# yuw444/fastF

Hardware: AMD Instinct MI355X
Metric: BAM records/sec -> deduped UMI matrix; achieved HBM GB/s vs roofline (higher is better)
Workload: dtype u64

## Files before the change

### fastf_amd/csrc/umi_engine.hip

```cpp
#include "umi_kernels.hpp"
#include "sweep_kernels.hpp"
#include "cap_kernels.hpp"

#include <algorithm>
#include <cstdarg>
#include <cstdio>
#include <cstdlib>
#include <cstring>
#include <mutex>
#include <new>
#include <stdexcept>
#include <chrono>
#include <string>
#include <thread>
#include <vector>

extern "C" {
#include "fastf_amd.h"
#include "host_io.h"
#include "mt_jump.h"
}

using namespace fastf;

// ... 173 lines not shown
    u64 batch_cap = 0;
    struct Slot {
        void* h_stage = nullptr;
        void* h_draws = nullptr;
        DevBuf d_stage;
        hipEvent_t ev_copy = nullptr, ev_done = nullptr;
        u64* h_small = nullptr;
        bool busy = false; u64 n = 0; bool external = false;
    } slot[2];
    int cur = 0;
    const u32* cur_umi_ext = nullptr;
    u64 inflight_records = 0;
    u64 key_cap = 0;
    DevBuf d_keys, d_tmp;
    DevBuf d_small;
    u64* h_small = nullptr;
    DevBuf d_feature, d_cell, d_count, d_ukeys, d_ncopy;
    u32* h_coo = nullptr; u64 h_coo_cap = 0, h_nnz = 0;
    bool h_coo_pinned = false; u32 h_coo_uses = 0;
    u32* lent_rows = nullptr; u64 lent_cap = 0;
    u32* rows_at = nullptr; u64 rows_stride = 0;
    std::vector<u32> h_ufeature, h_ucell, h_uumi, h_ncopy;
    std::vector<uint8_t> h_unonnull;
    u64 total_records = 0, hits_so_far = 0, keys_so_far = 0;
    u64 c_sampled = 0, c_valid = 0;
    bool finished = false; int sorted_in_tmp = 0; u64 n_sorted = 0;
    u32 skip_bits = 0;
    bool fully_sorted = false;
    DevBuf d_cellidx, d_tilecnt, d_tilebase, d_binbase, d_cnt;
    DevBuf d_halfhits;
    DevBuf d_segkeys;
    DevBuf d_segcount, d_segprefix, d_tileseg;
    u32 giant_parity = 0;
    u32 seg_n = 0; u64 seg_stride = 0;
    DevBuf d_rgn_phys, d_rgn_hist, d_rgn_blk;
    u32 rgn_hist_n = 0, rgn_hist_shift = 0;
    bool stream_mode = false, store_regions = false;
    bool narrow = false, genes_one_family = false;
    u64 slots_used = 0, slot_cap = 0; u32 rgn_n = 0, rgn_cap = 0;
    DevBuf d_scanblk;
    DevBuf d_rg_feature, d_rg_cell, d_rg_count, d_rg_ukeys, d_spanrows, d_spanbase, d_giant;
    u32 rg_n = 0; bool rg_umi = false;
    bool wide = false, long_umi = false; u32 group_bits = 0;
    u32 sub_bits = 0, row_split = 0;
    bool finish_queued = false;
    DevBuf d_vals, d_vtmp;
    bool timing = false;
    hipEvent_t t_ev[2] = {nullptr, nullptr};
    double t_scatter_ms = 0; u64 t_scatter_n = 0;
    double t_k1_ms = 0; u64 t_k1_n = 0;
    double t_k1b_ms = 0; u64 t_k1b_n = 0;
    double t_k3_ms = 0; u64 t_k3_n = 0;
    double t_count_ms = 0; u64 t_count_n = 0;
    double t_gather_ms = 0; u64 t_gather_n = 0;
};

enum { SM_KEYCOUNT = 0, SM_COUNTERS = 32, SM_NNZ = 64, SM_NROWS_U = 65, SM_N = 66, SM_RUNNING = 96, SM_DRAWBASE = 128, SM_WORDS = 160 };

static int set_scatter_lds_limit();
static u32 g_cu_count = 256;
static int multi_create(const fastf_engine_config_t* cfg, fastf_engine* e);
static void multi_destroy(fastf_engine* e);
static int multi_push(fastf_engine* e, const fastf_batch_t* b, bool pinned);
static int multi_finish(fastf_engine* e, fastf_coo_t* coo, uint64_t counters[3]);
static int multi_umi_rows(fastf_engine* e, fastf_umi_rows_t* rows);
static int multi_reset(fastf_engine* e, bool reseed, u32 seed, u64 skip);
static int multi_device_records(const fastf_engine* e, uint64_t* records, u32 n);
static size_t scatter_smem_bytes(u32 ipt = SORT_IPT) {
    return (size_t)ipt * SORT_THREADS * 8 + (size_t)SORT_WAVES * RADIX * 4 + RADIX * 4 * 2 + 64;
}

static u32 h_slot_hash(u64 key) {
    const u32 h = (u32)key * 0x9E3779B1u + (u32)(key >> 32) * 0x85EBCA77u;
    return h ^ (h >> 15);
}

static int build_table(const u64* keys, u32 n, DevBuf& buf, Table& t, const char* what) {
    u32 cap = 64;
    while (cap < 2ull * n) cap <<= 1;
    std::vector<uint4> slots(cap, make_uint4(0, 0, 0, 0));
    for (u32 i = 0; i < n; ++i) {
        const u64 k = keys[i];
        if (k == 0) return set_err("%s key %u is 0 (unpackable string?)", what, i);
        u32 h = h_slot_hash(k) & (cap - 1);
        for (;;) {
            uint4& s = slots[h];
            const u64 sk = ((u64)s.y << 32) | s.x;
            if (sk == 0) { s.x = (u32)k; s.y = (u32)(k >> 32); s.z = i + 1; break; }
            if (sk == k) return set_err("duplicate %s key at index %u (first occurrence wins in the reference; dedup before create)", what, i);
// ... 248 lines not shown
        int prio_lo = 0, prio_hi = 0;
        const char* sp = getenv("FASTF_STREAM_PRIORITY");
        const bool high = sp && sp[0] == '1' && hipDeviceGetStreamPriorityRange(&prio_lo, &prio_hi) == hipSuccess && prio_hi != prio_lo;
        auto mk = [&](hipStream_t* s) { return high ? hipStreamCreateWithPriority(s, hipStreamNonBlocking, prio_hi) : hipStreamCreateWithFlags(s, hipStreamNonBlocking); };
        if (mk(&e->s_compute) != hipSuccess ||
            mk(&e->s_copy) != hipSuccess ||
            mk(&e->s_mt) != hipSuccess ||
            hipEventCreateWithFlags(&e->ev_mt, hipEventDisableTiming) != hipSuccess ||
            hipEventCreateWithFlags(&e->slot[0].ev_copy, hipEventDisableTiming) != hipSuccess ||
            hipEventCreateWithFlags(&e->slot[1].ev_copy, hipEventDisableTiming) != hipSuccess ||
            hipEventCreateWithFlags(&e->slot[0].ev_done, hipEventDisableTiming) != hipSuccess ||
            hipEventCreateWithFlags(&e->slot[1].ev_done, hipEventDisableTiming) != hipSuccess ||
            hipEventCreate(&e->t_ev[0]) != hipSuccess || hipEventCreate(&e->t_ev[1]) != hipSuccess) {
            rc = set_err("stream/event creation failed"); break;
        }
        lap("streams and events");
        if ((rc = build_table((const u64*)cfg->cell_keys, cfg->n_cells, e->tab_cells, e->cells, "cell"))) break;
        if ((rc = build_table((const u64*)cfg->feature_keys, cfg->n_features, e->tab_feats, e->feats, "feature"))) break;
        {
            const char* lt = getenv("FASTF_LDS_TABLES");
            if (!(lt && lt[0] == '0')) {
                const char* lc = getenv("FASTF_LDS_CELLS");
                if (!(lc && lc[0] == '0') && (rc = build_cell_lds(e, (const u64*)cfg->cell_keys, cfg->n_cells))) break;
                if (!e->use_lds_cells && (rc = build_cell_filter(e, (const u64*)cfg->cell_keys, cfg->n_cells))) break;
                if ((rc = build_gene_lds(e, (const u64*)cfg->feature_keys, cfg->n_features))) break;
            }
        }
        lap("tables built and uploaded");
        if ((rc = e->d_small.ensure(SM_WORDS * sizeof(u64)))) break;
        if (hipHostMalloc((void**)&e->h_small, SM_WORDS * sizeof(u64), hipHostMallocDefault) != hipSuccess) {
            rc = set_err("hipHostMalloc failed"); break;
        }
        if (hipMemset(e->d_small.p, 0, SM_WORDS * sizeof(u64)) != hipSuccess) { rc = set_err("memset failed"); break; }
        lap("counters allocated and cleared");
        if (set_scatter_lds_limit()) {
            rc = set_err("cannot raise dynamic LDS limit to %zu bytes", scatter_smem_bytes()); break;
        }
        lap("kernel attributes (code object loaded)");
        e->batch_cap = cfg->batch_records ? cfg->batch_records : (4ull << 20);
        e->key_cap = cfg->key_capacity;
        e->stream_mode = e->use_lds_genes && !e->wide && e->n_shards == 1 && !getenv("FASTF_NO_STREAM_K1B") && !getenv("FASTF_PUSH_TILE_FORM");
        {
            const char* bw = getenv("FASTF_BLOCK_WIDE");
            e->narrow = e->stream_mode && e->genes_one_family && e->lds_genes.vmin + e->lds_genes.range <= 0xFFFFFFFFull &&
                        e->L.umi_bits <= 24 && !(bw && bw[0] == '1');
        }
    } while (0);
    if (rc) { fastf_engine_destroy(e); return 1; }
    *out = e;
    return 0;
} FASTF_CATCH_INT

extern "C" void fastf_engine_destroy(fastf_engine_t* e) FASTF_TRY {
    if (!e) return;
    if (e->multi) { multi_destroy(e); delete e; return; }
    (void)hipSetDevice(e->device);
    (void)hipDeviceSynchronize();
    for (int i = 0; i < 2; ++i) {
        fastf_engine::Slot& sl = e->slot[i];
        if (sl.h_stage) (void)hipHostFree(sl.h_stage);
        if (sl.h_draws) (void)hipHostFree(sl.h_draws);
        if (sl.h_small) (void)hipHostFree(sl.h_small);
        sl.d_stage.release();
        if (sl.ev_copy) (void)hipEventDestroy(sl.ev_copy);
        if (sl.ev_done) (void)hipEventDestroy(sl.ev_done);
        if (e->t_ev[i]) (void)hipEventDestroy(e->t_ev[i]);
    }
    if (e->h_small) (void)hipHostFree(e->h_small);
    if (e->h_coo) { if (e->h_coo_pinned) pin_unreg(e->h_coo); fastf_big_free(e->h_coo, (size_t)e->h_coo_cap * 12); }
    e->d_ring.release(); e->d_mt.release(); e->d_dbits.release(); e->d_mtwords.release(); e->d_mtsub.release(); e->d_mtpoly.release(); e->d_mtseat.release(); e->d_mtseq.release();
    DevBuf* all[] = {&e->tab_cells, &e->tab_feats, &e->img_cells, &e->img_genes, &e->d_cell_filter, &e->d_keys, &e->d_tmp, &e->d_small, &e->d_feature, &e->d_cell,
                     &e->d_count, &e->d_ukeys, &e->d_ncopy, &e->d_cellidx, &e->d_tilecnt, &e->d_tilebase, &e->d_binbase, &e->d_cnt, &e->d_rg_feature, &e->d_rg_cell, &e->d_rg_count, &e->d_rg_ukeys, &e->d_spanrows, &e->d_spanbase, &e->d_giant, &e->d_scanblk,
                     &e->d_halfhits, &e->d_segcount, &e->d_segprefix, &e->d_tileseg, &e->d_segkeys, &e->d_vals, &e->d_vtmp,
                     &e->d_rgn_phys, &e->d_rgn_hist, &e->d_rgn_blk};
    for (DevBuf* b : all) b->release();
    if (e->s_compute) (void)hipStreamDestroy(e->s_compute);
    if (e->s_copy) (void)hipStreamDestroy(e->s_copy);
    if (e->s_mt) (void)hipStreamDestroy(e->s_mt);
    if (e->ev_mt) (void)hipEventDestroy(e->ev_mt);
    delete e;
} FASTF_CATCH_VOID

extern "C" int fastf_engine_table_modes(const fastf_engine_t* e, int* cells_in_lds, int* genes_in_lds) FASTF_TRY {
    if (!e) return set_err("null engine");
    if (cells_in_lds) *cells_in_lds = e->use_lds_cells;
    if (genes_in_lds) *genes_in_lds = e->use_lds_genes ? (e->lds_genes.direct ? 2 : 1) : 0;
    return 0;
} FASTF_CATCH_INT

extern "C" int fastf_engine_cell_scratch_bytes(const fastf_engine_t* e, uint32_t* bytes) FASTF_TRY {
    if (!e || !bytes) return set_err("null argument");
    *bytes = (e->multi ? e->n_cells <= 65535u : e->cell16) ? 2u : 4u;
    return 0;
} FASTF_CATCH_INT

extern "C" int fastf_engine_sort_passes(const fastf_engine_t* e, uint32_t flags, uint32_t* passes) FASTF_TRY {
    if (!e || !passes) return set_err("null argument");
    *passes = sort_passes(e->L.total_bits, (flags & FASTF_SORT_SKIP_LOW) ? e->skip_bits : 0);
    return 0;
} FASTF_CATCH_INT

extern "C" int fastf_engine_skip_bits(const fastf_engine_t* e, uint32_t* bits) FASTF_TRY {
    if (!e || !bits) return set_err("null argument");
    *bits = e->skip_bits;
    return 0;
} FASTF_CATCH_INT

// ... 455 lines not shown
    p.keys = keys; p.shard_stride = stride; p.key_counts = key_counts; p.counters = counters;
    p.stamps = g_k1_stamps;
    p.n_tiles = tiles;
    p.genes = e->lds_genes;
    p.blk = (const unsigned char*)blk;
    if (e->wide) {
        if (segmented || blk) return set_err("internal error: wide keys take the tile form");
        if (!wide_vals && (e->n_shards != 1 || keys != (u64*)e->d_keys.p)) return set_err("internal error: wide keys go through the engine's own key store");
        p.vals = wide_vals ? wide_vals : (u64*)e->d_vals.p; p.wide_feat_bits = e->feat_bits; p.wide_sub_bits = e->sub_bits;
        p.umi_ext = wide_vals ? wide_ext : e->cur_umi_ext;
    }
    const bool no_stream = getenv("FASTF_NO_STREAM_K1B") != nullptr;
    const bool stream_shards = !segmented && !e->wide && e->n_shards > 1 && e->n_shards <= (u32)MAX_SHARDS && e->use_lds_genes && !no_stream;
    if (blk && !(segmented || stream_shards)) return set_err("FASTF_PROBE_BLOCKED needs the streaming K1b (fastf_dev_block_bytes returns 0 otherwise)");
    t_begin(e, s);
    if (segmented || stream_shards) {
        u32 grid; u64 region;
        stream_geometry(e, tiles, &grid, &region);
        const u32 n_rgn = grid * (u32)K1S_SUB, rgn0 = app ? app->rgn0 : 0u;
        if (stream_shards) {
            if (e->d_segkeys.ensure((size_t)n_rgn * region * sizeof(u64))) return 1;
            p.keys = (u64*)e->d_segkeys.p;
        } else if ((u64)n_rgn * region > stride) return set_err("segmented key output needs %llu slots, the buffer has %llu (fastf_dev_probe_capacity)",
                                                                (unsigned long long)((u64)n_rgn * region), (unsigned long long)stride);
        if (app) {
            if (e->rgn_cap < rgn0 + n_rgn) return set_err("internal error: region tables too small");
        } else {
            if (e->rgn_n) return set_err("device-level K1 on an engine that holds pushed chunks: fastf_engine_reset first");
            if (grow_regions(e, n_rgn)) return 1;
        }
        if (e->d_segprefix.ensure(((size_t)n_rgn + 1) * sizeof(u64))) return 1;
        StreamParams sp{(const u32*)e->d_halfhits.p, region, (u64*)e->d_segcount.p + rgn0,
                        stream_shards ? nullptr : (u32*)e->d_rgn_hist.p + (size_t)rgn0 * RADIX, (u64*)e->d_rgn_phys.p + rgn0,
                        app ? app->slot0 : 0ull, e->skip_bits};
        const int variant = (e->genes_blocks_per_cu >= 2 ? 0 : 4) | (e->cell16 ? 2 : 0) | (e->lds_genes.direct ? 1 : 0);
#define FPS(R, C, D) do { if (blk && e->narrow) hipLaunchKernelGGL((filter_pack_stream_kernel<R, C, D, true, true>), dim3(grid), dim3(R ? K1S_THREADS_ROOMY : K1S_THREADS), e->lds_genes.bytes, s, p, sp); \
                          else if (blk) hipLaunchKernelGGL((filter_pack_stream_kernel<R, C, D, true>), dim3(grid), dim3(R ? K1S_THREADS_ROOMY : K1S_THREADS), e->lds_genes.bytes, s, p, sp); \
                          else hipLaunchKernelGGL((filter_pack_stream_kernel<R, C, D, false>), dim3(grid), dim3(R ? K1S_THREADS_ROOMY : K1S_THREADS), e->lds_genes.bytes, s, p, sp); } while (0)
        switch (variant) {
        case 0: FPS(false, false, false); break; case 1: FPS(false, false, true); break;
        case 2: FPS(false, true, false); break;  case 3: FPS(false, true, true); break;
        case 4: FPS(true, false, false); break;  case 5: FPS(true, false, true); break;
        case 6: FPS(true, true, false); break;   default: FPS(true, true, true); break;
        }
#undef FPS
        if (stream_shards) {
            hipLaunchKernelGGL(shard_partition_kernel, dim3(n_rgn), dim3(SP_THREADS), 0, s, (const u64*)e->d_segkeys.p, (const u64*)e->d_segcount.p,
                               region, e->L.cell_shift, e->n_shards, keys, stride, key_counts, counters + 3);
        } else if (app) {
            hipLaunchKernelGGL(seg_scan_kernel, dim3(1), dim3(1024), 0, s, (const u64*)e->d_segcount.p + rgn0, n_rgn, (u64*)e->d_segprefix.p, key_counts, true);
        } else {
            hipLaunchKernelGGL(seg_scan_kernel, dim3(1), dim3(1024), 0, s, (const u64*)e->d_segcount.p, n_rgn, (u64*)e->d_segprefix.p, key_counts, false);
            e->seg_n = n_rgn; e->seg_stride = region;
            e->rgn_hist_n = n_rgn; e->rgn_hist_shift = e->skip_bits;
        }
    } else if (e->use_lds_genes) {
        const u32 grid = std::min<u32>(tiles, e->genes_blocks_per_cu * g_cu_count);
        if (e->genes_blocks_per_cu >= 2) hipLaunchKernelGGL((filter_pack_kernel<true, false>), dim3(grid), dim3(K1B_THREADS), e->lds_genes.bytes, s, p);
        else hipLaunchKernelGGL((filter_pack_kernel<true, true>), dim3(grid), dim3(K1B_THREADS), e->lds_genes.bytes, s, p);
    } else {
        hipLaunchKernelGGL(filter_pack_kernel<false>, dim3(tiles), dim3(K1B_THREADS), 0, s, p);
    }
    HIP_OK(hipGetLastError());
    t_end(e, s, &e->t_k1b_ms, &e->t_k1b_n);
    dbg_sync(s, blk ? "K1b filter_pack (blocked)" : "K1b filter_pack");
    return 0;
}

extern "C" int fastf_dev_probe_pack(fastf_engine_t* e, const uint64_t* d_cb_key, const uint64_t* d_gx_key,
                                    const uint32_t* d_umi, const uint32_t* d_meta, uint64_t n,
                                    const uint32_t* d_draws, uint64_t n_draws, const uint64_t* d_draw_base,
                                    uint64_t* d_keys_out, uint64_t shard_stride, uint64_t* d_key_counts,
                                    uint64_t* d_counters, uint32_t flags, void* stream) FASTF_TRY {
    if (!e) return set_err("null engine");
    if (e->multi) return set_err("fastf_dev_probe_pack: device-level calls take a single-device engine");
    HIP_OK(hipSetDevice(e->device));
    NO_WIDE(e, "fastf_dev_probe_pack");
    const bool seg = (flags & FASTF_PROBE_SEGMENTED) != 0, blocked = (flags & FASTF_PROBE_BLOCKED) != 0;
    if (seg && !(e->n_shards == 1 && e->use_lds_genes))
        return set_err("FASTF_PROBE_SEGMENTED needs a single shard and the gene table in LDS (fastf_dev_probe_capacity returns 0 otherwise)");
    if (blocked && !d_gx_key) return set_err("FASTF_PROBE_BLOCKED: d_gx_key must point at the blocked buffer");
    if (n && n_draws && !d_draws) return set_err("null d_draws");
    if (!(flags & FASTF_PROBE_DRAW_BITS) && n && n_draws) {
        if (e->d_dbits.ensure(((n_draws + 63) / 64) * 8)) return 1;
        if (launch_draw_bits(e->threshold, d_draws, n_draws, (u32*)e->d_dbits.p, (hipStream_t)stream)) return 1;
        d_draws = (const uint32_t*)e->d_dbits.p;
// ... 73 lines not shown

static int set_scatter_lds_limit() {
    const void* fns[10] = {(const void*)scatter_kernel<0>, (const void*)scatter_kernel<8>, (const void*)scatter_kernel<16>,
                           (const void*)scatter_kernel<24>, (const void*)scatter_kernel<32>, (const void*)scatter_kernel<40>,
                           (const void*)scatter_kernel<48>, (const void*)scatter_kernel<56>, (const void*)scatter_kernel<-1>,
                           (const void*)scatter_kernel<-1, true>};
    for (const void* f : fns)
        if (hipFuncSetAttribute(f, hipFuncAttributeMaxDynamicSharedMemorySize, (int)scatter_smem_bytes()) != hipSuccess) return 1;
    if (hipFuncSetAttribute((const void*)scatter_kernel<-1, false, true>, hipFuncAttributeMaxDynamicSharedMemorySize, (int)scatter_smem_bytes_vals(SORT_IPT)) != hipSuccess) return 1;
    if (hipFuncSetAttribute((const void*)scatter_regions_kernel, hipFuncAttributeMaxDynamicSharedMemorySize, (int)scatter_smem_bytes()) != hipSuccess) return 1;
    return 0;
}

static int launch_sort(fastf_engine* e, u64* keys, u64* tmp, const u64* d_n, u64 max_n, u32 key_bits, u32 low_bit,
                       int* sorted_in_tmp, hipStream_t s, bool segmented_input = false, u64* vals = nullptr, u64* vtmp = nullptr) {
    if (key_bits > 64) return set_err("key_bits %u > 64", key_bits);
    const u32 passes = sort_passes(key_bits, low_bit);
    *sorted_in_tmp = (int)(passes & 1);
    if (max_n == 0) return 0;
    if (max_n >= (1ull << 32)) return set_err("sort of %llu keys: limit is 2^32-1 per shard", (unsigned long long)max_n);
    if (reserve_workspace(e, 0, max_n)) return 1;
    const u32 ipt = choose_sort_ipt(max_n);
    const u32 T = (u32)((max_n + (u64)ipt * SORT_THREADS - 1) / ((u64)ipt * SORT_THREADS));
    u32* bintot = (u32*)e->d_binbase.p; u32* cnt = (u32*)e->d_cnt.p;
    SegMap seg{nullptr, nullptr, 0, 0};
    bool walk = false;
    if (segmented_input) {
        if (!e->seg_n) return set_err("FASTF_SORT_SEGMENTED without a preceding FASTF_PROBE_SEGMENTED probe_pack");
        if (passes == 0) return set_err("segmented keys need at least one sort pass");
        static const bool no_walk = getenv("FASTF_NO_REGION_WALK") != nullptr;
        walk = e->rgn_hist_n == e->seg_n && e->rgn_hist_shift == low_bit && !no_walk && !vals;
        if (!walk) {
            if (!e->seg_stride) return set_err("internal error: regions without a common stride need their histograms");
            seg = SegMap{(const u64*)e->d_segprefix.p, (const TileSeg*)e->d_tileseg.p, e->seg_n, e->seg_stride};
            hipLaunchKernelGGL(seg_tiles_kernel, dim3(std::min<u32>((T + 255) / 256, 1024)), dim3(256), 0, s, seg.prefix, seg.n_seg,
                               seg.stride, ipt * SORT_THREADS, (TileSeg*)e->d_tileseg.p);
        }
    }
    const SegMap none{nullptr, nullptr, 0, 0};
    for (u32 q = 0; q < passes; ++q) {
        const u64* src = (q & 1) ? tmp : keys;
        u64* dst = (q & 1) ? keys : tmp;
        const u32 shift = low_bit + 8 * q;
        if (q == 0 && walk) {
            const u32 R = e->seg_n, n_blk = (R + RGN_BLK - 1) / RGN_BLK;
            if (e->d_rgn_blk.ensure((size_t)n_blk * RADIX * sizeof(u32))) return 1;
            hipLaunchKernelGGL(rgn_scan_blocks_kernel, dim3(n_blk), dim3(RADIX), 0, s, (u32*)e->d_rgn_hist.p, R, (u32*)e->d_rgn_blk.p);
            hipLaunchKernelGGL(rgn_scan_fix_kernel, dim3(n_blk), dim3(RADIX), 0, s, (u32*)e->d_rgn_hist.p, R, (const u32*)e->d_rgn_blk.p, n_blk, bintot);
            t_begin(e, s);
            hipLaunchKernelGGL(scatter_regions_kernel, dim3(tile_grid(R)), dim3(SORT_THREADS), scatter_smem_bytes(ipt), s, src, dst,
                               (const u64*)e->d_rgn_phys.p, (const u64*)e->d_segcount.p, (const u32*)e->d_rgn_hist.p, (const u32*)bintot, R, ipt, shift,
                               max_n >= (24ull << 20));
            t_end(e, s, &e->t_scatter_ms, &e->t_scatter_n);
            e->rgn_hist_n = 0;
            dbg_sync(s, "K2 sort pass (region walk)");
            continue;
        }
        t_begin(e, s);
        if (q == 0 && seg.prefix) hipLaunchKernelGGL(tile_count_kernel<true>, dim3(tile_grid(T)), dim3(SORT_THREADS), 0, s, src, d_n, shift, cnt, ipt, seg);
        else hipLaunchKernelGGL(tile_count_kernel<false>, dim3(tile_grid(T)), dim3(SORT_THREADS), 0, s, src, d_n, shift, cnt, ipt, none);
        t_end(e, s, &e->t_count_ms, &e->t_count_n);
        hipLaunchKernelGGL(row_scan_kernel, dim3(RADIX), dim3(1024), 0, s, cnt, d_n, bintot, ipt);
        t_begin(e, s);
        if (vals) launch_scatter(shift, T, s, src, dst, d_n, (const u32*)cnt, (const u32*)bintot, ipt, none, (q & 1) ? vtmp : vals, (q & 1) ? vals : vtmp);
        else launch_scatter(shift, T, s, src, dst, d_n, (const u32*)cnt, (const u32*)bintot, ipt, q == 0 ? seg : none);
        t_end(e, s, &e->t_scatter_ms, &e->t_scatter_n);
        dbg_sync(s, "K2 sort pass");
    }
    HIP_OK(hipGetLastError());
    return 0;
}

extern "C" int fastf_dev_set_regions(fastf_engine_t* e, const uint64_t* d_counts, uint32_t n_regions, uint64_t stride,
                                     uint64_t* d_n_out, void* stream) FASTF_TRY {
    if (!e || !d_counts || !d_n_out) return set_err("null argument");
    if (e->multi) return set_err("fastf_dev_set_regions: device-level calls take a single-device engine");
    if (n_regions == 0 || stride == 0) return set_err("fastf_dev_set_regions: no regions");
    HIP_OK(hipSetDevice(e->device));
    if (e->d_segprefix.ensure(((size_t)n_regions + 1) * sizeof(u64))) return 1;
    hipLaunchKernelGGL(seg_scan_kernel, dim3(1), dim3(1024), 0, (hipStream_t)stream, (const u64*)d_counts, (u32)n_regions, (u64*)e->d_segprefix.p, (u64*)d_n_out);
    HIP_OK(hipGetLastError());
    e->seg_n = n_regions; e->seg_stride = stride; e->rgn_hist_n = 0;
    return 0;
} FASTF_CATCH_INT

extern "C" int fastf_dev_sort(fastf_engine_t* e, uint64_t* d_keys, uint64_t* d_tmp, const uint64_t* d_n,
                              uint64_t max_n, uint32_t key_bits, uint32_t flags, int* sorted_in_tmp, void* stream) FASTF_TRY {
    if (!e) return set_err("null engine");
    if (e->multi) return set_err("fastf_dev_sort: device-level calls take a single-device engine");
    NO_WIDE(e, "fastf_dev_sort");
    HIP_OK(hipSetDevice(e->device));
    int dummy = 0;
    return launch_sort(e, (u64*)d_keys, (u64*)d_tmp, (const u64*)d_n, max_n, key_bits,
                       (flags & FASTF_SORT_SKIP_LOW) ? e->skip_bits : 0,
                       sorted_in_tmp ? sorted_in_tmp : &dummy, (hipStream_t)stream, (flags & FASTF_SORT_SEGMENTED) != 0);
} FASTF_CATCH_INT

static u32 k3_grid(u64 max_n, int dedup) {
    static int per_cu[3] = {-1, -1, -1};
    if (per_cu[dedup] < 0) {
        const char* c = getenv("FASTF_K3_PER_CU");
        per_cu[dedup] = c ? atoi(c) : 4;
        if (per_cu[dedup] < 1) per_cu[dedup] = 1;
    }
    const u64 tiles = (max_n + K3_TILE - 1) / K3_TILE;
    return (u32)std::min<u64>(std::max<u64>(tiles, 1), std::min<u64>((u64)per_cu[dedup] * g_cu_count, 4096));
}

template <bool UMI_ROWS>
static int launch_reduce_regions(fastf_engine* e, const u64* sorted, const u64* d_n, u64 max_n, u64* nrows, u32 low_skip, hipStream_t s,
                                 const u64* wide_vals = nullptr) {
    e->rg_n = 0;
    if (max_n == 0) { HIP_OK(hipMemsetAsync(nrows, 0, sizeof(u64), s)); return 0; }
    if (wide_vals && UMI_ROWS) return set_err("internal error: -u rows of wide keys");
    const int dedup = wide_vals ? 2 : (UMI_ROWS || low_skip == 0) ? 0 : 2;
// ... 876 lines not shown
```

### fastf_amd/csrc/umi_kernels.hpp

```cpp
#pragma once
#if !defined(FASTF_EXPERIMENT)
#  if defined(FASTF_X_ANY)
#    error "FASTF_X_* knobs need -DFASTF_EXPERIMENT (experiment builds only: tools/build_variant.sh)"
#  endif
#endif
#ifndef FASTF_K1_IPT
#define FASTF_K1_IPT 8
#endif
#ifndef FASTF_K1_THREADS
#define FASTF_K1_THREADS 512
#endif
#include <hip/hip_runtime.h>
#include <stdint.h>
#include <type_traits>

namespace fastf {

typedef unsigned long long u64;
typedef unsigned int u32;

constexpr int WAVE = 64;

constexpr u64 ERR_DRAWS_SHORT  = 2;
constexpr u64 ERR_UMI_TOOLONG  = 4;
// ... 879 lines not shown
    if (tid == 0) s_err = 0;
    if constexpr (LDS_GENES) {
        __syncthreads();
        for (u32 tile = blockIdx.x; tile < p.n_tiles; tile += gridDim.x) {
            do_tile(tile);
            __syncthreads();
        }
    } else {
        __syncthreads();
        do_tile(blockIdx.x);
        __syncthreads();
    }
    if (tid < 3 && s_tot[tid]) atomicAdd(&p.counters[tid], s_tot[tid]);
    if (tid == 3 && s_err) atomicOr(&p.counters[3], (u64)s_err);
}

constexpr int K1S_IPT = 4, K1S_UNIT = K1S_IPT * WAVE;
static_assert(K1_TILE % K1S_UNIT == 0 && K1_TILE / K1S_UNIT == 16, "16 units per K1a tile");
#ifndef FASTF_K1S_THREADS
#define FASTF_K1S_THREADS 768
#endif
constexpr int K1S_THREADS = FASTF_K1S_THREADS, K1S_THREADS_ROOMY = 1024;
static_assert(K1S_THREADS % (4 * WAVE) == 0 && K1S_THREADS <= 1024, "whole waves on every SIMD");

constexpr int K1S_SUB = 2, K1S_BINS = 256;
struct StreamParams {
    const u32* half_hits;
    u64 region_stride;
    u64* seg_count;
    u32* rgn_hist;
    u64* rgn_phys;
    u64 slot0;
    u32 hist_shift;
};

__device__ __forceinline__ u32 row16_sum_lane15(u32 x) {
    x += (u32)__builtin_amdgcn_update_dpp(0, (int)x, 0x111, 0xF, 0xF, true);
    x += (u32)__builtin_amdgcn_update_dpp(0, (int)x, 0x112, 0xF, 0xF, true);
    x += (u32)__builtin_amdgcn_update_dpp(0, (int)x, 0x114, 0xF, 0xF, true);
    x += (u32)__builtin_amdgcn_update_dpp(0, (int)x, 0x118, 0xF, 0xF, true);
    return (u32)__builtin_amdgcn_readlane((int)x, 15);
}

template <bool ROOMY, bool C16, bool DIRECT, bool BLOCKED = false, bool NARROW = false>
__global__ __launch_bounds__(ROOMY ? K1S_THREADS_ROOMY : K1S_THREADS, ROOMY ? 4 : 2 * K1S_THREADS / (4 * WAVE)) void filter_pack_stream_kernel(const PackParams p, const StreamParams sp) {
    static_assert(BLOCKED || !NARROW, "the narrow records exist as blocked runs only");
    constexpr int THREADS = ROOMY ? K1S_THREADS_ROOMY : K1S_THREADS, WAVES = THREADS / WAVE;
    __shared__ u64 s_tot[3];
    __shared__ u32 s_cursor[K1S_SUB], s_err;
    __shared__ u32 s_hist[K1S_SUB * K1S_BINS];
    extern __shared__ __attribute__((aligned(16))) unsigned char smem[];
    const int tid = threadIdx.x, lane = lane_id();
    const int w = __builtin_amdgcn_readfirstlane(tid >> 6);
    const u32* s_bitmap = reinterpret_cast<const u32*>(smem);
    const unsigned short* s_rank = reinterpret_cast<const unsigned short*>(smem + (size_t)p.genes.words * 4);
    const unsigned short* s_perm = s_rank + ((p.genes.words + 1u) & ~1u);
    const unsigned short* s_direct = reinterpret_cast<const unsigned short*>(smem);
    {
        const uint4* src = reinterpret_cast<const uint4*>(p.genes.image);
        uint4* dst = reinterpret_cast<uint4*>(smem);
        for (u32 i = tid; i < (p.genes.bytes + 15u) / 16u; i += THREADS) dst[i] = src[i];
    }
    if (tid < 3) s_tot[tid] = 0;
    if (tid < K1S_SUB) s_cursor[tid] = 0;
    if (tid == 0) s_err = 0;
    for (int i = tid; i < K1S_SUB * K1S_BINS; i += THREADS) s_hist[i] = 0;
// ... 169 lines not shown
                    pos0 += (u32)__popcll(em[j]);
                }
            }
        }
        u = un;
    };
    while (u < n_units) {
        one_unit(ra, rb, std::integral_constant<int, 0>{});
        if (u >= n_units) break;
        one_unit(rb, ra, std::integral_constant<int, 1>{});
    }
    if (lane == 0) {
        if (w_hit) atomicAdd(&s_tot[0], (u64)w_hit);
        if (w_samp) atomicAdd(&s_tot[1], (u64)w_samp);
        if (w_valid) atomicAdd(&s_tot[2], (u64)w_valid);
    }
    {
        u32 e = errs;
#pragma unroll
        for (int o = 32; o > 0; o >>= 1) e |= __shfl_xor(e, o, WAVE);
        if (lane == 0 && e) atomicOr(&s_err, e);
    }
    __syncthreads();
    const int te = w * WAVE + lane;
    if (te < 3 && s_tot[te]) atomicAdd(&p.counters[te], s_tot[te]);
    if (te == 3 && s_err) atomicOr(&p.counters[3], (u64)s_err);
    if (te >= 64 && te < 64 + K1S_SUB) {
        const u32 r = blockIdx.x * K1S_SUB + (u32)(te - 64);
        sp.seg_count[r] = s_cursor[te - 64];
        if (sp.rgn_hist) sp.rgn_phys[r] = sp.slot0 + (u64)r * sp.region_stride;
    }
    if (sp.rgn_hist)
        for (int i = te; i < K1S_SUB * K1S_BINS; i += THREADS) sp.rgn_hist[(u64)blockIdx.x * (K1S_SUB * K1S_BINS) + i] = s_hist[i];
}

template <bool NARROW>
__global__ __launch_bounds__(256) void block_records_kernel(const u64* __restrict__ gx, const u32* __restrict__ umi, const u32* __restrict__ meta,
                                                            u64 n, unsigned char* __restrict__ blk, u32 run, u32 family, const KeyLayout L) {
    const u64 units = (n + BLK_RECS - 1) / BLK_RECS, waves = (u64)gridDim.x * (blockDim.x / WAVE);
    const int lane = lane_id();
    for (u64 u = (u64)blockIdx.x * (blockDim.x / WAVE) + (threadIdx.x >> 6); u < units; u += waves) {
        unsigned char* const r = blk + u * run;
#pragma unroll
        for (int j = 0; j < (int)BLK_RECS / WAVE; ++j) {
            const u32 o = (u32)j * WAVE + (u32)lane;
            const u64 i = u * BLK_RECS + o;
            const bool in = i < n;
            if constexpr (NARROW) {
                const u64 k = in ? gx[i] : 0;
                const u32 um = in ? umi[i] : 0, me = in ? meta[i] : 0;
                const u64 v = k & 0xFFFFFFFFFFFull;
                reinterpret_cast<u32*>(r + NBLK_GX)[o] = ((k != 0) & ((u32)(k >> 44) == family) & (v < 0xFFFFFFFFull)) ? (u32)v + 1u : 0u;
                reinterpret_cast<u32*>(r + NBLK_UM)[o] = (um & ~0xFFu) | (me & 0xFFu) | (umi_overflows_flat(L, um, me) ? META_UMI_TOOLONG : 0u);
            } else {
                reinterpret_cast<u64*>(r + BLK_GX)[o] = in ? gx[i] : 0;
                reinterpret_cast<u32*>(r + BLK_UMI)[o] = in ? umi[i] : 0;
                reinterpret_cast<u32*>(r + BLK_META)[o] = in ? meta[i] : 0;
            }
        }
    }
}

constexpr int SP_THREADS = 256, SP_IPT = 8, SP_TILE = SP_THREADS * SP_IPT, MAX_SHARDS = 8;
__global__ __launch_bounds__(SP_THREADS) void shard_partition_kernel(const u64* __restrict__ seg_keys, const u64* __restrict__ seg_count,
                                                                     u64 region_stride, u32 cell_shift, u32 n_shards,
                                                                     u64* __restrict__ keys_out, u64 shard_stride,
// ... 26 lines not shown
        for (int j = 0; j < SP_IPT; ++j) {
            const u64 i = i0 + (u64)j * SP_THREADS + tid;
            if (i < cnt && s_base[sh[j]] != ~0ull) keys_out[(u64)sh[j] * shard_stride + s_base[sh[j]] + lp[j]] = key[j];
        }
        __syncthreads();
    }
}

struct TileSeg { u64 delta1, hi1, delta2, hi2; };
struct SegMap { const u64* prefix; const TileSeg* tile_seg; u32 n_seg; u64 stride; };

__global__ __launch_bounds__(1024) void seg_scan_kernel(const u64* __restrict__ seg_count, u32 n_seg, u64* __restrict__ prefix,
                                                        u64* __restrict__ n_out, bool add = false) {
    __shared__ u64 s_w[16];
    __shared__ u64 s_carry;
    const int lane = lane_id(), w = threadIdx.x >> 6;
    if (threadIdx.x == 0) s_carry = 0;
    __syncthreads();
    for (u32 b0 = 0; b0 < n_seg; b0 += 1024) {
        const u32 b = b0 + threadIdx.x;
        const u64 v = b < n_seg ? seg_count[b] : 0;
        u64 inc = v;
#pragma unroll
        for (int o = 1; o < WAVE; o <<= 1) { const u64 x = __shfl_up(inc, o, WAVE); if (lane >= o) inc += x; }
        if (lane == WAVE - 1) s_w[w] = inc;
        __syncthreads();
        u64 off = s_carry;
        for (int i = 0; i < w; ++i) off += s_w[i];
        if (b < n_seg) prefix[b] = off + inc - v;
        __syncthreads();
        if (threadIdx.x == 1023) s_carry = off + inc;
        __syncthreads();
    }
    if (threadIdx.x == 0) { prefix[n_seg] = s_carry; *n_out = add ? *n_out + s_carry : s_carry; }
}

__device__ __forceinline__ u32 seg_region_of(const u64* __restrict__ prefix, u32 n_seg, u64 idx) {
    u32 lo = 0, hi = n_seg;
    while (hi - lo > 1) { const u32 mid = (lo + hi) >> 1; if (prefix[mid] <= idx) lo = mid; else hi = mid; }
    return lo;
}

__global__ __launch_bounds__(256) void seg_tiles_kernel(const u64* __restrict__ prefix, u32 n_seg, u64 stride, u32 tile_keys,
                                                        TileSeg* __restrict__ tile_seg) {
    const u64 total = prefix[n_seg];
    const u64 T = (total + tile_keys - 1) / tile_keys;
    for (u64 t = (u64)blockIdx.x * 256 + threadIdx.x; t < T; t += (u64)gridDim.x * 256) {
        const u64 first = t * tile_keys;
        const u32 b = seg_region_of(prefix, n_seg, first);
        TileSeg ts;
        ts.delta1 = (u64)b * stride - prefix[b]; ts.hi1 = prefix[b + 1];
        u32 b2 = b + 1;
        while (b2 < n_seg && prefix[b2 + 1] == ts.hi1) ++b2;
        if (b2 < n_seg) { ts.delta2 = (u64)b2 * stride - prefix[b2]; ts.hi2 = prefix[b2 + 1]; }
        else { ts.delta2 = 0; ts.hi2 = ts.hi1; }
        tile_seg[t] = ts;
    }
}

__device__ __forceinline__ u64 seg_phys(const SegMap m, u64 idx, const TileSeg ts) {
    if (idx < ts.hi1) return idx + ts.delta1;
    if (idx < ts.hi2) return idx + ts.delta2;
    const u32 b = seg_region_of(m.prefix, m.n_seg, idx);
    return (u64)b * m.stride + (idx - m.prefix[b]);
}

constexpr int RADIX = 256;
// ... 82 lines not shown
        if (q * 4 >= T) v.x = 0;
        const u32 sum = v.x + v.y + v.z + v.w;
        const u32 inc = wave_incl_scan32(sum, lane);
        if (lane == WAVE - 1) s_w[w] = inc;
        __syncthreads();
        u32 off = s_carry;
        for (int i = 0; i < w; ++i) off += s_w[i];
        const u32 e0 = off + inc - sum;
        if (q * 4 < T) row[q] = make_uint4(e0, e0 + v.x, e0 + v.x + v.y, e0 + v.x + v.y + v.z);
        __syncthreads();
        if (threadIdx.x == 1023) s_carry = off + inc;
        __syncthreads();
    }
    if (threadIdx.x == 0) bin_tot[blockIdx.x] = s_carry;
}

__device__ __forceinline__ void match_digit(u32 d, u32& mlo, u32& mhi) {
    mlo = ~0u; mhi = ~0u;
#pragma unroll
    for (int b = 0; b < 8; ++b) {
        const int ext = __builtin_amdgcn_sbfe((int)d, b, 1);
        const u64 bal = __builtin_amdgcn_ballot_w64(ext != 0);
        mlo = __builtin_amdgcn_bitop3_b32(mlo, (u32)bal, (u32)ext, 0x90);
        mhi = __builtin_amdgcn_bitop3_b32(mhi, (u32)(bal >> 32), (u32)ext, 0x90);
    }
}

template <int SHIFT>
__device__ __forceinline__ u32 digit_of(u64 key, u32 rshift) {
    if constexpr (SHIFT >= 0) return (u32)(key >> SHIFT) & 255u;
    else return (u32)(key >> rshift) & 255u;
}

template <int SHIFT, bool FULL, bool SEG, bool VALS = false>
__device__ __forceinline__ u32 scatter_tile(const u64* __restrict__ in, u64* __restrict__ out, u64 base, u32 n_valid,
                                            u32 tile, const u32 g_off, const u32* __restrict__ bin_tot,
                                            const int ipt, unsigned char* smem, const u32 rshift, const SegMap seg, const int tid,
                                            const bool streams, u64* stamps = nullptr,
                                            const u64* __restrict__ vin = nullptr, u64* __restrict__ vout = nullptr) {
#ifdef FASTF_STAMPS
#define STAMP(i) do { if (stamps && threadIdx.x == 0) stamps[(u64)tile * 8 + (i)] = __builtin_amdgcn_s_memtime(); } while (0)
#else
#define STAMP(i) do { } while (0)
#endif
    STAMP(0);
    u64* s_keys = reinterpret_cast<u64*>(smem);
    u32* s_whist = reinterpret_cast<u32*>(smem + (size_t)ipt * SORT_THREADS * 8);
    u32* s_delta = s_whist + SORT_WAVES * RADIX;
    u32* s_start = s_delta + RADIX;
    u32* s_wtot  = s_start + RADIX;
    u64* s_vals  = reinterpret_cast<u64*>(s_wtot + 16);
    const int lane = tid & (WAVE - 1), w = tid >> 6;

    for (int i = tid; i < SORT_WAVES * RADIX; i += SORT_THREADS) s_whist[i] = 0;
    const u32 g_tot = tid < RADIX ? bin_tot[tid] : 0u;

    u64 key[SORT_IPT];
    const u32 wbase = (u32)w * (u32)ipt * WAVE;
    if constexpr (SEG) {
        const TileSeg ts = seg.tile_seg[tile];
#pragma unroll
        for (int j = 0; j < SORT_IPT; ++j) {
            const u32 li = wbase + j * WAVE + lane;
            key[j] = (j < ipt && (FULL || li < n_valid)) ? ld_once<FASTF_NT_SORT != 0>(in + seg_phys(seg, base + li, ts)) : ~0ULL;
        }
    } else if (streams) {
#pragma unroll
        for (int j = 0; j < SORT_IPT; ++j) {
            const u32 li = wbase + j * WAVE + lane;
            key[j] = (j < ipt && (FULL || li < n_valid)) ? ld_once<FASTF_NT_SORT != 0>(in + base + li) : ~0ULL;
        }
    } else {
#pragma unroll
        for (int j = 0; j < SORT_IPT; ++j) {
            const u32 li = wbase + j * WAVE + lane;
            key[j] = (j < ipt && (FULL || li < n_valid)) ? in[base + li] : ~0ULL;
        }
    }
    u64 val[SORT_IPT];
    if constexpr (VALS) {
#pragma unroll
        for (int j = 0; j < SORT_IPT; ++j) {
            const u32 li = wbase + j * WAVE + lane;
            val[j] = (j < ipt && (FULL || li < n_valid)) ? vin[base + li] : 0;
        }
    }
    __syncthreads();
#ifdef FASTF_STAMPS
// ... 85 lines not shown
    const bool streams = sort_streams(n);
    for (u32 r = blockIdx.x >> 3;; r += gridDim.x >> 3) {
#ifdef FASTF_NO_XCD_SWIZZLE
        const u32 tile = (r << 3) | (blockIdx.x & 7u);
#else
        const u32 tile = xcd_tile(T, r);
#endif
        if (tile >= T) return;
        const u64 base = (u64)tile * tile_keys;
        const u32 n_valid = (u32)((n - base) < (u64)tile_keys ? (n - base) : (u64)tile_keys);
        int tid = (int)threadIdx.x;
        asm volatile("" : "+v"(tid));
        const u32 g_off = tid < RADIX ? off[(u64)tid * row_stride(T) + tile] : 0u;
        if (n_valid == tile_keys) (void)scatter_tile<SHIFT, true, SEG, VALS>(in, out, base, n_valid, tile, g_off, bin_tot, (int)ipt, smem, rshift, seg, tid, streams, stamps, vin, vout);
        else (void)scatter_tile<SHIFT, false, SEG, VALS>(in, out, base, n_valid, tile, g_off, bin_tot, (int)ipt, smem, rshift, seg, tid, streams, stamps, vin, vout);
        if constexpr (VALS) __syncthreads();
    }
}

constexpr u32 RGN_BLK = 64;
static_assert(K1S_BINS == RADIX, "K1b's region histograms are histograms of a sort digit");
__global__ __launch_bounds__(RADIX) void rgn_scan_blocks_kernel(u32* __restrict__ hist, u32 R, u32* __restrict__ blk_sum) {
    const u32 d = threadIdx.x, r0 = blockIdx.x * RGN_BLK, r1 = r0 + RGN_BLK < R ? r0 + RGN_BLK : R;
    u32 acc = 0;
    for (u32 r = r0; r < r1; r += 8) {
        u32 v[8];
#pragma unroll
        for (u32 k = 0; k < 8; ++k) v[k] = r + k < r1 ? hist[(u64)(r + k) * RADIX + d] : 0u;
#pragma unroll
        for (u32 k = 0; k < 8; ++k) { if (r + k < r1) hist[(u64)(r + k) * RADIX + d] = acc; acc += v[k]; }
    }
    blk_sum[(u64)blockIdx.x * RADIX + d] = acc;
}
__global__ __launch_bounds__(RADIX) void rgn_scan_fix_kernel(u32* __restrict__ hist, u32 R, const u32* __restrict__ blk_sum, u32 n_blk,
                                                             u32* __restrict__ bin_tot) {
    const u32 d = threadIdx.x, w = blockIdx.x;
    u32 off = 0, tot = 0;
    for (u32 i = 0; i < n_blk; ++i) { const u32 v = blk_sum[(u64)i * RADIX + d]; off += i < w ? v : 0u; tot += v; }
    if (w == 0) bin_tot[d] = tot;
    if (off == 0) return;
    const u32 r0 = w * RGN_BLK, r1 = r0 + RGN_BLK < R ? r0 + RGN_BLK : R;
    for (u32 r = r0; r < r1; ++r) hist[(u64)r * RADIX + d] += off;
}
__global__ __launch_bounds__(SORT_THREADS, 8) void scatter_regions_kernel(const u64* __restrict__ keys, u64* __restrict__ out,
                                                                           const u64* __restrict__ rgn_phys, const u64* __restrict__ rgn_count,
                                                                           const u32* __restrict__ hist_excl, const u32* __restrict__ bin_tot,
                                                                           u32 R, u32 ipt, u32 rshift, bool streams) {
    extern __shared__ __attribute__((aligned(16))) unsigned char smem[];
    const u32 tile_keys = ipt * SORT_THREADS;
    const SegMap none{nullptr, nullptr, 0, 0};
    for (u32 i = blockIdx.x >> 3;; i += gridDim.x >> 3) {
        const u32 r = xcd_tile(R, i);
        if (r >= R) return;
        const u64 cnt = rgn_count[r];
        const u64* const in = keys + rgn_phys[r];
        u32 acc = threadIdx.x < RADIX ? hist_excl[(u64)r * RADIX + threadIdx.x] : 0u;
        for (u64 base = 0; base < cnt; base += tile_keys) {
            const u32 n_valid = (u32)(cnt - base < (u64)tile_keys ? cnt - base : (u64)tile_keys);
            int tid = (int)threadIdx.x;
            asm volatile("" : "+v"(tid));
            u32 run;
            if (n_valid == tile_keys) run = scatter_tile<-1, true, false>(in, out, base, n_valid, r, acc, bin_tot, (int)ipt, smem, rshift, none, tid, streams);
            else run = scatter_tile<-1, false, false>(in, out, base, n_valid, r, acc, bin_tot, (int)ipt, smem, rshift, none, tid, streams);
            acc += run;
        }
    }
}
__global__ __launch_bounds__(256) void rgn_hist_kernel(const u64* __restrict__ keys, const u64* __restrict__ rgn_phys, const u64* __restrict__ rgn_count,
                                                       u32 R, u32 shift, u32* __restrict__ hist) {
    __shared__ u32 s_h[RADIX];
    for (u32 r = blockIdx.x; r < R; r += gridDim.x) {
        s_h[threadIdx.x] = 0;
        __syncthreads();
        const u64 cnt = rgn_count[r];
        const u64* const in = keys + rgn_phys[r];
        for (u64 i = threadIdx.x; i < cnt; i += 256) atomicAdd(&s_h[(u32)(in[i] >> shift) & 255u], 1u);
        __syncthreads();
        hist[(u64)r * RADIX + threadIdx.x] = s_h[threadIdx.x];
        __syncthreads();
    }
}


struct ReduceParams {
    const u64* keys; const u64* n_ptr;
    KeyLayout L; u32 feat_mask;
    u64* err;
    u32* feature; u32* cell; u32* count;
    u64* ukeys;
    u32* span_rows;
    u64* giant_list; u32* giant_n;
    u32 giant_max;
    const u64* vals; u32 wide_feat_bits;
};

constexpr u32 GIANT_MAX = 1u << 16, GIANT_PART = 1536, GIANT_LIST_CAP = 4096, GIANT_ITEM_WORDS = 4, GIANT_TAB = 4096;
// ... 643 lines not shown
```

Before: 107.8 billion.

## Fold segment scan and region-scan fixup into neighbouring kernels

The single-block seg_scan launch after the K1b filter/pack kernel is replaced by a last-block-done ticket that sums per-block counts atomically and writes the key count. The segment prefix scan is deferred and only run lazily when the non-walk sort path needs it. The rgn_scan_fix kernel is removed: each scatter block now sums the per-block histogram totals itself to get its offset and the global bin totals. This removes launches and serial single-block work, at the cost of extra atomics and redundant per-block reads of blk_sum.

```diff
diff --git a/fastf_amd/csrc/umi_engine.hip b/fastf_amd/csrc/umi_engine.hip
--- a/fastf_amd/csrc/umi_engine.hip
+++ b/fastf_amd/csrc/umi_engine.hip
@@ -229,6 +229,8 @@
     DevBuf d_segkeys;
     DevBuf d_segcount, d_segprefix, d_tileseg;
     u32 giant_parity = 0;
+    bool seg_prefix_ok = false;
+    DevBuf d_fin;
     u32 seg_n = 0; u64 seg_stride = 0;
     DevBuf d_rgn_phys, d_rgn_hist, d_rgn_blk;
     u32 rgn_hist_n = 0, rgn_hist_shift = 0;
@@ -252,6 +254,7 @@
     double t_gather_ms = 0; u64 t_gather_n = 0;
 };
 
+enum { FIN_K1B = 0, FIN_LINES = 4 };
 enum { SM_KEYCOUNT = 0, SM_COUNTERS = 32, SM_NNZ = 64, SM_NROWS_U = 65, SM_N = 66, SM_RUNNING = 96, SM_DRAWBASE = 128, SM_WORDS = 160 };
 
 static int set_scatter_lds_limit();
@@ -566,6 +569,8 @@
             rc = set_err("hipHostMalloc failed"); break;
         }
         if (hipMemset(e->d_small.p, 0, SM_WORDS * sizeof(u64)) != hipSuccess) { rc = set_err("memset failed"); break; }
+        if ((rc = e->d_fin.ensure(FIN_LINES * 128))) break;
+        if (hipMemset(e->d_fin.p, 0, FIN_LINES * 128) != hipSuccess) { rc = set_err("memset failed"); break; }
         lap("counters allocated and cleared");
         if (set_scatter_lds_limit()) {
             rc = set_err("cannot raise dynamic LDS limit to %zu bytes", scatter_smem_bytes()); break;
@@ -606,7 +611,7 @@
     DevBuf* all[] = {&e->tab_cells, &e->tab_feats, &e->img_cells, &e->img_genes, &e->d_cell_filter, &e->d_keys, &e->d_tmp, &e->d_small, &e->d_feature, &e->d_cell,
                      &e->d_count, &e->d_ukeys, &e->d_ncopy, &e->d_cellidx, &e->d_tilecnt, &e->d_tilebase, &e->d_binbase, &e->d_cnt, &e->d_rg_feature, &e->d_rg_cell, &e->d_rg_count, &e->d_rg_ukeys, &e->d_spanrows, &e->d_spanbase, &e->d_giant, &e->d_scanblk,
                      &e->d_halfhits, &e->d_segcount, &e->d_segprefix, &e->d_tileseg, &e->d_segkeys, &e->d_vals, &e->d_vtmp,
-                     &e->d_rgn_phys, &e->d_rgn_hist, &e->d_rgn_blk};
+                     &e->d_rgn_phys, &e->d_rgn_hist, &e->d_rgn_blk, &e->d_fin};
     for (DevBuf* b : all) b->release();
     if (e->s_compute) (void)hipStreamDestroy(e->s_compute);
     if (e->s_copy) (void)hipStreamDestroy(e->s_copy);
@@ -1128,7 +1133,8 @@
         if (e->d_segprefix.ensure(((size_t)n_rgn + 1) * sizeof(u64))) return 1;
         StreamParams sp{(const u32*)e->d_halfhits.p, region, (u64*)e->d_segcount.p + rgn0,
                         stream_shards ? nullptr : (u32*)e->d_rgn_hist.p + (size_t)rgn0 * RADIX, (u64*)e->d_rgn_phys.p + rgn0,
-                        app ? app->slot0 : 0ull, e->skip_bits};
+                        app ? app->slot0 : 0ull, e->skip_bits,
+                        stream_shards ? nullptr : (StreamParams::Fin*)((char*)e->d_fin.p + FIN_K1B * 128), app ? 1u : 0u};
         const int variant = (e->genes_blocks_per_cu >= 2 ? 0 : 4) | (e->cell16 ? 2 : 0) | (e->lds_genes.direct ? 1 : 0);
 #define FPS(R, C, D) do { if (blk && e->narrow) hipLaunchKernelGGL((filter_pack_stream_kernel<R, C, D, true, true>), dim3(grid), dim3(R ? K1S_THREADS_ROOMY : K1S_THREADS), e->lds_genes.bytes, s, p, sp); \
                           else if (blk) hipLaunchKernelGGL((filter_pack_stream_kernel<R, C, D, true>), dim3(grid), dim3(R ? K1S_THREADS_ROOMY : K1S_THREADS), e->lds_genes.bytes, s, p, sp); \
@@ -1143,11 +1149,8 @@
         if (stream_shards) {
             hipLaunchKernelGGL(shard_partition_kernel, dim3(n_rgn), dim3(SP_THREADS), 0, s, (const u64*)e->d_segkeys.p, (const u64*)e->d_segcount.p,
                                region, e->L.cell_shift, e->n_shards, keys, stride, key_counts, counters + 3);
-        } else if (app) {
-            hipLaunchKernelGGL(seg_scan_kernel, dim3(1), dim3(1024), 0, s, (const u64*)e->d_segcount.p + rgn0, n_rgn, (u64*)e->d_segprefix.p, key_counts, true);
-        } else {
-            hipLaunchKernelGGL(seg_scan_kernel, dim3(1), dim3(1024), 0, s, (const u64*)e->d_segcount.p, n_rgn, (u64*)e->d_segprefix.p, key_counts, false);
-            e->seg_n = n_rgn; e->seg_stride = region;
+        } else if (!app) {
+            e->seg_n = n_rgn; e->seg_stride = region; e->seg_prefix_ok = false;
             e->rgn_hist_n = n_rgn; e->rgn_hist_shift = e->skip_bits;
         }
     } else if (e->use_lds_genes) {
@@ -1287,6 +1290,11 @@
         walk = e->rgn_hist_n == e->seg_n && e->rgn_hist_shift == low_bit && !no_walk && !vals;
         if (!walk) {
             if (!e->seg_stride) return set_err("internal error: regions without a common stride need their histograms");
+            if (!e->seg_prefix_ok) {
+                if (e->d_segprefix.ensure(((size_t)e->seg_n + 1) * sizeof(u64))) return 1;
+                hipLaunchKernelGGL(seg_scan_kernel, dim3(1), dim3(1024), 0, s, (const u64*)e->d_segcount.p, e->seg_n, (u64*)e->d_segprefix.p, (u64*)nullptr, false);
+                e->seg_prefix_ok = true;
+            }
             seg = SegMap{(const u64*)e->d_segprefix.p, (const TileSeg*)e->d_tileseg.p, e->seg_n, e->seg_stride};
             hipLaunchKernelGGL(seg_tiles_kernel, dim3(std::min<u32>((T + 255) / 256, 1024)), dim3(256), 0, s, seg.prefix, seg.n_seg,
                                seg.stride, ipt * SORT_THREADS, (TileSeg*)e->d_tileseg.p);
@@ -1301,10 +1309,9 @@
             const u32 R = e->seg_n, n_blk = (R + RGN_BLK - 1) / RGN_BLK;
             if (e->d_rgn_blk.ensure((size_t)n_blk * RADIX * sizeof(u32))) return 1;
             hipLaunchKernelGGL(rgn_scan_blocks_kernel, dim3(n_blk), dim3(RADIX), 0, s, (u32*)e->d_rgn_hist.p, R, (u32*)e->d_rgn_blk.p);
-            hipLaunchKernelGGL(rgn_scan_fix_kernel, dim3(n_blk), dim3(RADIX), 0, s, (u32*)e->d_rgn_hist.p, R, (const u32*)e->d_rgn_blk.p, n_blk, bintot);
             t_begin(e, s);
             hipLaunchKernelGGL(scatter_regions_kernel, dim3(tile_grid(R)), dim3(SORT_THREADS), scatter_smem_bytes(ipt), s, src, dst,
-                               (const u64*)e->d_rgn_phys.p, (const u64*)e->d_segcount.p, (const u32*)e->d_rgn_hist.p, (const u32*)bintot, R, ipt, shift,
+                               (const u64*)e->d_rgn_phys.p, (const u64*)e->d_segcount.p, (const u32*)e->d_rgn_hist.p, (const u32*)e->d_rgn_blk.p, n_blk, R, ipt, shift,
                                max_n >= (24ull << 20));
             t_end(e, s, &e->t_scatter_ms, &e->t_scatter_n);
             e->rgn_hist_n = 0;
@@ -1335,7 +1342,7 @@
     if (e->d_segprefix.ensure(((size_t)n_regions + 1) * sizeof(u64))) return 1;
     hipLaunchKernelGGL(seg_scan_kernel, dim3(1), dim3(1024), 0, (hipStream_t)stream, (const u64*)d_counts, (u32)n_regions, (u64*)e->d_segprefix.p, (u64*)d_n_out);
     HIP_OK(hipGetLastError());
-    e->seg_n = n_regions; e->seg_stride = stride; e->rgn_hist_n = 0;
+    e->seg_n = n_regions; e->seg_stride = stride; e->rgn_hist_n = 0; e->seg_prefix_ok = true;
     return 0;
 } FASTF_CATCH_INT
 
diff --git a/fastf_amd/csrc/umi_kernels.hpp b/fastf_amd/csrc/umi_kernels.hpp
--- a/fastf_amd/csrc/umi_kernels.hpp
+++ b/fastf_amd/csrc/umi_kernels.hpp
@@ -935,6 +935,9 @@
     u64* rgn_phys;
     u64 slot0;
     u32 hist_shift;
+    struct Fin { u32 ticket, pad; u64 acc; };
+    Fin* fin;
+    u32 n_add;
 };
 
 __device__ __forceinline__ u32 row16_sum_lane15(u32 x) {
@@ -1170,6 +1173,18 @@
     }
     if (sp.rgn_hist)
         for (int i = te; i < K1S_SUB * K1S_BINS; i += THREADS) sp.rgn_hist[(u64)blockIdx.x * (K1S_SUB * K1S_BINS) + i] = s_hist[i];
+    if (sp.fin && te == 2 * WAVE) {
+        u64 mine = 0;
+#pragma unroll
+        for (int k = 0; k < K1S_SUB; ++k) mine += s_cursor[k];
+        if (mine) (void)__hip_atomic_fetch_add(&sp.fin->acc, mine, __ATOMIC_RELAXED, __HIP_MEMORY_SCOPE_AGENT);
+        const u32 ticket = __hip_atomic_fetch_add(&sp.fin->ticket, 1u, __ATOMIC_ACQ_REL, __HIP_MEMORY_SCOPE_AGENT);
+        if (ticket == gridDim.x - 1u) {
+            const u64 total = __hip_atomic_exchange(&sp.fin->acc, 0ull, __ATOMIC_RELAXED, __HIP_MEMORY_SCOPE_AGENT);
+            __hip_atomic_store(&sp.fin->ticket, 0u, __ATOMIC_RELAXED, __HIP_MEMORY_SCOPE_AGENT);
+            p.key_counts[0] = sp.n_add ? p.key_counts[0] + total : total;
+        }
+    }
 }
 
 template <bool NARROW>
@@ -1262,7 +1277,7 @@
         if (threadIdx.x == 1023) s_carry = off + inc;
         __syncthreads();
     }
-    if (threadIdx.x == 0) { prefix[n_seg] = s_carry; *n_out = add ? *n_out + s_carry : s_carry; }
+    if (threadIdx.x == 0) { prefix[n_seg] = s_carry; if (n_out) *n_out = add ? *n_out + s_carry : s_carry; }
 }
 
 __device__ __forceinline__ u32 seg_region_of(const u64* __restrict__ prefix, u32 n_seg, u64 idx) {
@@ -1411,12 +1426,13 @@
     else return (u32)(key >> rshift) & 255u;
 }
 
-template <int SHIFT, bool FULL, bool SEG, bool VALS = false>
+template <int SHIFT, bool FULL, bool SEG, bool VALS = false, bool GTOT = false>
 __device__ __forceinline__ u32 scatter_tile(const u64* __restrict__ in, u64* __restrict__ out, u64 base, u32 n_valid,
                                             u32 tile, const u32 g_off, const u32* __restrict__ bin_tot,
                                             const int ipt, unsigned char* smem, const u32 rshift, const SegMap seg, const int tid,
                                             const bool streams, u64* stamps = nullptr,
-                                            const u64* __restrict__ vin = nullptr, u64* __restrict__ vout = nullptr) {
+                                            const u64* __restrict__ vin = nullptr, u64* __restrict__ vout = nullptr,
+                                            const u32 g_tot_in = 0u) {
 #ifdef FASTF_STAMPS
 #define STAMP(i) do { if (stamps && threadIdx.x == 0) stamps[(u64)tile * 8 + (i)] = __builtin_amdgcn_s_memtime(); } while (0)
 #else
@@ -1432,7 +1448,8 @@
     const int lane = tid & (WAVE - 1), w = tid >> 6;
 
     for (int i = tid; i < SORT_WAVES * RADIX; i += SORT_THREADS) s_whist[i] = 0;
-    const u32 g_tot = tid < RADIX ? bin_tot[tid] : 0u;
+    u32 g_tot;
+    if constexpr (GTOT) g_tot = g_tot_in; else g_tot = tid < RADIX ? bin_tot[tid] : 0u;
 
     u64 key[SORT_IPT];
     const u32 wbase = (u32)w * (u32)ipt * WAVE;
@@ -1584,19 +1601,9 @@
     }
     blk_sum[(u64)blockIdx.x * RADIX + d] = acc;
 }
-__global__ __launch_bounds__(RADIX) void rgn_scan_fix_kernel(u32* __restrict__ hist, u32 R, const u32* __restrict__ blk_sum, u32 n_blk,
-                                                             u32* __restrict__ bin_tot) {
-    const u32 d = threadIdx.x, w = blockIdx.x;
-    u32 off = 0, tot = 0;
-    for (u32 i = 0; i < n_blk; ++i) { const u32 v = blk_sum[(u64)i * RADIX + d]; off += i < w ? v : 0u; tot += v; }
-    if (w == 0) bin_tot[d] = tot;
-    if (off == 0) return;
-    const u32 r0 = w * RGN_BLK, r1 = r0 + RGN_BLK < R ? r0 + RGN_BLK : R;
-    for (u32 r = r0; r < r1; ++r) hist[(u64)r * RADIX + d] += off;
-}
 __global__ __launch_bounds__(SORT_THREADS, 8) void scatter_regions_kernel(const u64* __restrict__ keys, u64* __restrict__ out,
                                                                            const u64* __restrict__ rgn_phys, const u64* __restrict__ rgn_count,
-                                                                           const u32* __restrict__ hist_excl, const u32* __restrict__ bin_tot,
+                                                                           const u32* __restrict__ hist_excl, const u32* __restrict__ blk_sum, u32 n_blk,
                                                                            u32 R, u32 ipt, u32 rshift, bool streams) {
     extern __shared__ __attribute__((aligned(16))) unsigned char smem[];
     const u32 tile_keys = ipt * SORT_THREADS;
@@ -1606,14 +1613,19 @@
         if (r >= R) return;
         const u64 cnt = rgn_count[r];
         const u64* const in = keys + rgn_phys[r];
-        u32 acc = threadIdx.x < RADIX ? hist_excl[(u64)r * RADIX + threadIdx.x] : 0u;
+        u32 acc = 0, g_tot = 0;
+        if (threadIdx.x < RADIX) {
+            acc = hist_excl[(u64)r * RADIX + threadIdx.x];
+            const u32 wb = r / RGN_BLK;
+            for (u32 b = 0; b < n_blk; ++b) { const u32 v = blk_sum[(u64)b * RADIX + threadIdx.x]; acc += b < wb ? v : 0u; g_tot += v; }
+        }
         for (u64 base = 0; base < cnt; base += tile_keys) {
             const u32 n_valid = (u32)(cnt - base < (u64)tile_keys ? cnt - base : (u64)tile_keys);
             int tid = (int)threadIdx.x;
             asm volatile("" : "+v"(tid));
             u32 run;
-            if (n_valid == tile_keys) run = scatter_tile<-1, true, false>(in, out, base, n_valid, r, acc, bin_tot, (int)ipt, smem, rshift, none, tid, streams);
-            else run = scatter_tile<-1, false, false>(in, out, base, n_valid, r, acc, bin_tot, (int)ipt, smem, rshift, none, tid, streams);
+            if (n_valid == tile_keys) run = scatter_tile<-1, true, false, false, true>(in, out, base, n_valid, r, acc, nullptr, (int)ipt, smem, rshift, none, tid, streams, nullptr, nullptr, nullptr, g_tot);
+            else run = scatter_tile<-1, false, false, false, true>(in, out, base, n_valid, r, acc, nullptr, (int)ipt, smem, rshift, none, tid, streams, nullptr, nullptr, nullptr, g_tot);
             acc += run;
         }
     }
```

Result: no change. 107.3 billion (-0.5%).
